# ShamG1/marl-traffic-intersection

Hardware: AMD Instinct MI355X
Metric: agent-steps/sec (whole node) at 4096 envs × 8 agents × 64-beam lidar; 1/2/4/8 GPU (higher is better)
Workload: dtype f32

## Files before the change

marl-traffic-intersection_amd/csrc/mev_kernels.hip:

```cpp
#include <type_traits>

#include <cstdlib>

#include "mev_kernels.h"
#include "mev_world.h"
#include "mev_nsort.h"

namespace mev {

#ifdef MEV_STAMPS
#define STAMP_RAW(k)                                                     \
    do {                                                                 \
        __builtin_amdgcn_wave_barrier();                                 \
        if (threadIdx.x == 0) p.debug[e * 8 + (k)] = __builtin_amdgcn_s_memtime(); \
    } while (0)
#if defined(MEV_STAMPS_R)
#undef STAMP_RAW
#define STAMP_RAW(k)                                                     \
    do {                                                                 \
        __builtin_amdgcn_wave_barrier();                                 \
        if (threadIdx.x == 0) p.debug[e * 8 + (k)] = __builtin_amdgcn_s_memrealtime(); \
    } while (0)
#ifndef MEV_STAMPS_POSTEND
#define MEV_STAMPS_POSTEND 0
// ... 2041 lines not shown
                                  float iady, float rwm, float ccen, float crf) {
    const float big = 1.0e6f;
    const float rx = fx - 375.0f, ry = fy - 375.0f;
    const float ax = fabs_f(rx), ay = fabs_f(ry);
    const float sx = ax < rwm ? rwm * iadx - rx * idx : 0.0f;
    const float sy = ay < rwm ? rwm * iady - ry * idy : 0.0f;
    const float sqm = ccen - 1.55f, rg = crf + 2.0f;
    const float qx = rx != 0.0f ? rx : dx, qy = ry != 0.0f ? ry : dy;
    const float ocx = rx - (qx >= 0.0f ? ccen : -ccen), ocy = ry - (qy >= 0.0f ? ccen : -ccen);
    const float bq = ocx * dx + ocy * dy;
    const float cq = ocx * ocx + ocy * ocy - rg * rg;
    const float disc = bq * bq - cq;
    const float troot = lidar_keep(-bq - __builtin_amdgcn_sqrtf(disc));
    const float tdisc = cq <= 0.0f ? 0.0f : ((disc < 0.0f || bq >= 0.0f) ? big : troot);
    const float tsq = fminf(sqm * iadx - rx * idx, sqm * iady - ry * idy);
    const float tq = fminf(rx * dx < 0.0f ? -rx * idx : big, ry * dy < 0.0f ? -ry * idy : big);
    const float sc = fmaxf(ax, ay) < sqm ? fminf(tdisc, fminf(tsq, tq)) : 0.0f;
    const float road = fmaxf(fmaxf(sx, sy), sc);
    const float tx = (dx > 0.0f ? 748.5f - fx : fx - 0.5f) * iadx;
    const float ty = (dy > 0.0f ? 748.5f - fy : fy - 0.5f) * iady;
    return fminf(road, fminf(tx, ty));
}

__device__ inline float road_safe_uniform(float fx, float fy, float dx, float dy, float idx, float idy, float iadx,
                                          float iady, float rwm, float ccen, float crf) {
    const float big = 1.0e6f;
    const float rx = fx - 375.0f, ry = fy - 375.0f;
    const float ax = fabs_f(rx), ay = fabs_f(ry);
    const float sqm = ccen - 1.55f, rg = crf + 2.0f;
    float road = 0.0f;
    if (__builtin_amdgcn_readfirstlane((int)(ax < rwm))) road = fmaxf(road, rwm * iadx - rx * idx);
    if (__builtin_amdgcn_readfirstlane((int)(ay < rwm))) road = fmaxf(road, rwm * iady - ry * idy);
    if (__builtin_amdgcn_readfirstlane((int)(fmaxf(ax, ay) < sqm))) {
        const float qx = rx != 0.0f ? rx : dx, qy = ry != 0.0f ? ry : dy;
        const float ocx = rx - (qx >= 0.0f ? ccen : -ccen), ocy = ry - (qy >= 0.0f ? ccen : -ccen);
        const float bq = ocx * dx + ocy * dy;
        const float cq = ocx * ocx + ocy * ocy - rg * rg;
        const float disc = bq * bq - cq;
        const float troot = lidar_keep(-bq - __builtin_amdgcn_sqrtf(disc));
        const float tdisc = cq <= 0.0f ? 0.0f : ((disc < 0.0f || bq >= 0.0f) ? big : troot);
        const float tsq = fminf(sqm * iadx - rx * idx, sqm * iady - ry * idy);
        const float tq = fminf(rx * dx < 0.0f ? -rx * idx : big, ry * dy < 0.0f ? -ry * idy : big);
        road = fmaxf(road, fminf(tdisc, fminf(tsq, tq)));
    }
    const float tx = (dx > 0.0f ? 748.5f - fx : fx - 0.5f) * iadx;
    const float ty = (dy > 0.0f ? 748.5f - fy : fy - 0.5f) * iady;
    return fminf(road, fminf(tx, ty));
}

__device__ inline float atan2_fast(float y, float x) {
    const float ax = fabs_f(x), ay = fabs_f(y);
    const float mx = fmaxf(ax, ay), mn = fminf(ax, ay);
    const float t = mn * __builtin_amdgcn_rcpf(fmaxf(mx, 1e-30f));
    const float s2 = t * t;
    float r = ((-0.0464964749f * s2 + 0.15931422f) * s2 - 0.327622764f) * s2 * t + t;
    r = ay > ax ? 1.57079637f - r : r;
    r = x < 0.0f ? 3.14159274f - r : r;
    return y < 0.0f ? -r : r;
}

__device__ inline float wrap_pi_fast(float a) { return a - 6.28318531f * rintf(a * 0.159154943f); }

__device__ inline float box_lo(int lo) { return (float)(lo > 0 ? lo : lo - 1) - 0.01f; }
__device__ inline float box_hi(int hi) { return (float)hi + 1.01f; }

__device__ inline void slab_clip(float c0, float dc, float idc, float a, float b, float& lo, float& hi) {
    if (fabs_f(dc) < 1e-6f) {
        if (c0 < a || c0 > b) { lo = 1.0f; hi = 0.0f; }
        return;
    }
    const float t1 = (a - c0) * idc, t2 = (b - c0) * idc;
    lo = fmaxf(lo, fminf(t1, t2));
    hi = fminf(hi, fmaxf(t1, t2));
}




#ifndef MEV_LIDAR_NPR
#define MEV_LIDAR_NPR 2
#endif
constexpr int LIDAR_NPR = MEV_LIDAR_NPR;
constexpr int kMarchHelp = 16;
constexpr int kNptHelp = 3;
static_assert(kMarchHelp <= 32, "helper groups have at least 2 lanes");

int lidar_group(int R) {
    int g = 256 / (R > 0 ? R : 1);
    return g < 1 ? 1 : (g > 64 ? 64 : g);
}

struct LidarSrcHbm {
    static constexpr bool kBoxLds = false;
    const SimParams& p;
    __device__ float rel(int b) const { return gmem(p.rel_angles)[b]; }
    __device__ bool alive(int g) const { return gmem(p.ego.alive)[g] != 0; }
    __device__ float4 pose(int g) const { return make_float4(egof(p, EF_X)[g], egof(p, EF_Y)[g], egof(p, EF_H)[g], __int_as_float(g)); }
    __device__ void cand(int g, unsigned long long& c0, unsigned long long& c1) const {
        c0 = gmem(p.ob_cand)[2 * g];
        c1 = gmem(p.ob_cand)[2 * g + 1];
    }
    __device__ int4 box(int g, int o) const { return p.ob_box[(size_t)(g / p.N) * p.ob_stride + o]; }
};
struct LidarSrcLds {
    static constexpr bool kBoxLds = true;
    const CarsLDS& el;
    int g0;
    __device__ float rel(int b) const { return el.rel[b]; }
    __device__ bool alive(int g) const { return el.alive[g - g0] != 0; }
    __device__ float4 pose(int g) const {
        const int i = g - g0;
        return make_float4(el.x[i], el.y[i], el.h[i], __int_as_float(g));
    }
    __device__ void cand(int g, unsigned long long& c0, unsigned long long& c1) const {
        c0 = el.cand[2 * (g - g0)];
        c1 = el.cand[2 * (g - g0) + 1];
    }
    __device__ int4 box(int, int o) const { return el.box[o]; }
};
template <int ENVS>
struct LidarSrcLdsEnvs {
    static constexpr bool kBoxLds = true;
    const CarsLDS& el0;
    int reg;
    const float* relp;
    int env[ENVS];
    __device__ int off(int g) const {
        int j = 0;
#pragma unroll
        for (int u = 1; u < ENVS; ++u) j = g == env[u] ? u : j;
        return j * reg;
    }
    template <class T>
    __device__ const T* at(const T* p0, int g) const {
        return reinterpret_cast<const T*>(reinterpret_cast<const unsigned char*>(p0) + off(g));
    }
    __device__ float rel(int b) const { return relp[b]; }
    __device__ bool alive(int g) const { return at(el0.alive, g)[0] != 0; }
    __device__ float4 pose(int g) const {
        return make_float4(at(el0.x, g)[0], at(el0.y, g)[0], at(el0.h, g)[0], __int_as_float(g));
    }
    __device__ void cand(int g, unsigned long long& c0, unsigned long long& c1) const {
        const unsigned long long* c = at(el0.cand, g);
        c0 = c[0];
        c1 = c[1];
    }
    __device__ int4 box(int g, int o) const { return at(el0.box, g)[o]; }
};

#ifndef MEV_DENSE_ILP
#define MEV_DENSE_ILP 2
#endif
template <bool TAB, int ILP, class Src, int NPT = LIDAR_NPR, bool HELP = false, int PART = 0, int P1 = 0,
          bool WC = false>
__device__ __forceinline__ void lidar_body(const SimParams& p, const Outputs& out, const Src& src, const int G,
                                           const int a0, const int na, const int lane, unsigned char* base,
                                           const LidarLayout& lay, const unsigned long long redo = 0ull,
                                           const unsigned long long alive_in = 0ull) {
    static_assert(!WC || (!TAB && P1 >= WAVE), "the reference's world: no distance table, the beams at compile time");
    using W = StepWorld<WC>;
    using RW = StepRows<WC, P1>;
    const int R = P1 >= WAVE ? P1 : p.R;
    const int LS = P1 >= WAVE ? P1 : p.lidar_slots;
    float4* ag = reinterpret_cast<float4*>(base + lay.ag);
    float2* dir = reinterpret_cast<float2*>(base + lay.dir);
    int* res = reinterpret_cast<int*>(base + lay.res);
#if defined(MEV_STAMPS_R)
    const int se_ = a0 / p.N, sp_ = ((a0 % p.N) / G) & 1;
    if (lane == 0) p.debug[se_ * 8 + 3 + sp_] = __builtin_amdgcn_s_memrealtime();
#endif

    bool alv = false;
    if (PART != 0) alv = (alive_in >> lane) & 1ull;
    else if (lane < na) alv = src.alive(a0 + lane);
    const unsigned long long am = PART != 0 ? alive_in : ballot(alv);
    const int nal = __popcll(am);
    if (PART == 0 && alv) {
        const int g = a0 + lane;
        ag[lane_rank(am)] = src.pose(g);
    }
    if (PART != 2 && __popcll(am) != na) {
        for (int j = 0; j < na; ++j) {
            if ((am >> j) & 1ull) continue;
            if (RW::lidar_u8(out)) {
                uint8_t* crow = RW::lidar_u8(out) + (size_t)(a0 + j) * LS;
                for (int b = lane; b < LS; b += WAVE) crow[b] = (uint8_t)kLidarCodeDead;
                continue;
            }
            float* row = out.obs + (size_t)(a0 + j) * RW::obs_ld(out) + OBS_HEAD;
            for (int b = lane; b < LS; b += WAVE) row[b] = 0.0f;
        }
    }
    wave_lds_sync();
    const float stp = W::lidar_step(p);
    const int S = W::lidar_steps(p);
    const float rwf = (float)W::irw(p);
    const float inv_stp = __builtin_amdgcn_rcpf(stp);
    const float crf = CORNER_RADIUS, ccen = rwf + crf;
    const float cr2p1 = crf * crf + 1.0f;
    const float rwm = rwf - 1.5f;
    auto probe = [&](float cx_, float cy_, float dx_, float dy_, int k_, float& fx, float& fy) -> int {
        const bool past = k_ >= S;
        const int kc = past ? S - 1 : k_;
        const float d = TAB ? gmem(p.dist_tab)[kc] : (float)kc * stp;
        fx = cx_ + dx_ * d;
        fy = cy_ + dy_ * d;
        const int px = (int)fx, py = (int)fy;
        const unsigned pmax = (unsigned)px > (unsigned)py ? (unsigned)px : (unsigned)py;
        const bool off_screen = pmax >= (unsigned)WIDTH;
        const float iax = fabs_f((float)(px - 375)), iay = fabs_f((float)(py - 375));
        const float qdx = iax - ccen, qdy = iay - ccen;
        const float onv = fmaxf(fminf(fminf(iax, iay) - rwf, fmaxf(iax, iay) - ccen), cr2p1 - (qdx * qdx + qdy * qdy));
        const bool stop = off_screen | ((k_ > 0) & (onv > 0.0f));
        const int code = lidar_keep(stop ? ((k_ << 1) | (off_screen ? 0 : 1)) : -1);
        return past ? (S << 1) : code;
    };
    auto probes_n = [&](auto np, float cx_, float cy_, float dx_, float dy_, int k_, float& fx, float& fy) -> int {
        int r = -1;
#pragma unroll
        for (int t = 0; t < decltype(np)::value; ++t) {
            const int c = probe(cx_, cy_, dx_, dy_, k_ + t, fx, fy);
            r = r >= 0 ? r : c;
        }
        return r;
    };
    auto probes = [&](float cx_, float cy_, float dx_, float dy_, int k_, float& fx, float& fy) -> int {
        return probes_n(std::integral_constant<int, LIDAR_NPR>{}, cx_, cy_, dx_, dy_, k_, fx, fy);
    };

    unsigned short* queue = reinterpret_cast<unsigned short*>(base + lay.queue);
    int qn = 0;
    const float rel_c0 = lane < R ? src.rel(lane) : 0.0f;
    const float rel_c1 = lane + WAVE < R ? src.rel(lane + WAVE) : 0.0f;
    auto setup = [&](const float4& a, float rel_b, auto small, float2& d, bool uni) -> int {
        float sn, cs;
#if defined(MEV_EXP_FASTSIN)
        sn = __sinf(a.z + rel_b);
        cs = __cosf(a.z + rel_b);
        (void)small;
#else
        if constexpr (decltype(small)::value) sincosf_below120(a.z + rel_b, &sn, &cs);
        else sincosf(a.z + rel_b, &sn, &cs);
#endif
        const float dx = cs, dy = -sn;
        d = make_float2(dx, dy);
        const int px = (int)a.x, py = (int)a.y;
        const unsigned pmax = (unsigned)px > (unsigned)py ? (unsigned)px : (unsigned)py;
        const float idx = __builtin_amdgcn_rcpf(dx), idy = __builtin_amdgcn_rcpf(dy);
        float safe;
        if (uni)
            safe = road_safe_uniform(a.x, a.y, dx, dy, idx, idy, fabs_f(idx), fabs_f(idy), rwm, ccen, crf);
        else
            safe = road_safe(a.x, a.y, dx, dy, idx, idy, fabs_f(idx), fabs_f(idy), rwm, ccen, crf);
        const int k1 = pmax < (unsigned)WIDTH ? 1 + safe_steps(safe, stp, inv_stp) : 0;
        float fx, fy;
        const int r = probes_n(std::integral_constant<int, LIDAR_NPR>{}, a.x, a.y, dx, dy, k1, fx, fy);
        return r >= 0 ? r : -(k1 + LIDAR_NPR) - 1;
    };
    auto pass1_one = [&](auto small, const int j) {
        const float4 a = ag[j];
        for (int b0 = 0; b0 < R; b0 += WAVE) {
            const int b = b0 + lane;
            const bool vb = b < R;
            const float rel_b = b0 == 0 ? rel_c0 : (b0 == WAVE ? rel_c1 : (vb ? src.rel(b) : 0.0f));
            float2 d;
            const int r = setup(a, rel_b, small, d, true);
            if (vb) {
                dir[j * R + b] = d;
                res[j * R + b] = r >= 0 ? r : -r - 1;
            }
            const bool pend = vb && r < 0;
            const unsigned long long m = ballot(pend);
            if (pend) queue[qn + lane_rank(m)] = (unsigned short)(j * R + b);
            qn += __popcll(m);
        }
    };
    const bool dense = P1 >= WAVE ? (P1 & (WAVE - 1)) != 0 : (P1 == 2 || (P1 == 0 && (R & (WAVE - 1)) != 0 && nal > 1));
    auto phase1 = [&](auto small) {
        if constexpr (PART == 2) {
            for (unsigned long long tm = redo; tm; tm &= tm - 1ull) pass1_one(small, __builtin_ctzll(tm));
        } else if (dense) {
            const float invRp = 1.0f / (float)R;
            const int nq = nal * R;
            constexpr int DI = ILP > 1 ? MEV_DENSE_ILP : 1;
            for (int c0 = 0; c0 < nq; c0 += DI * WAVE) {
                if (PART == 0 && 4 * c0 >= nq) __builtin_amdgcn_s_setprio(kPrioP1B);
                int q[DI];
                float4 a[DI];
                float rb[DI];
#pragma unroll
                for (int u = 0; u < DI; ++u) {
                    q[u] = c0 + u * WAVE + lane;
                    const int qc = q[u] < nq ? q[u] : nq - 1;
                    const int j = (int)(((float)qc + 0.5f) * invRp);
                    a[u] = ag[j];
                    rb[u] = src.rel(qc - j * R);
                }
                float2 d[DI];
                int r[DI];
#pragma unroll
                for (int u = 0; u < DI; ++u) r[u] = setup(a[u], rb[u], small, d[u], false);
#pragma unroll
                for (int u = 0; u < DI; ++u) {
                    const bool vq = q[u] < nq;
                    if (vq) {
                        dir[q[u]] = d[u];
                        res[q[u]] = r[u] >= 0 ? r[u] : -r[u] - 1;
// ... 8 lines not shown
        for (int j = 0; j < nal; j += ILP) {
            if (PART == 0 && 4 * j >= nal) __builtin_amdgcn_s_setprio(kPrioP1B);
            float4 a[ILP];
#pragma unroll
            for (int u = 0; u < ILP; ++u) a[u] = ag[j + u < nal ? j + u : j];
            for (int b0 = 0; b0 < R; b0 += WAVE) {
                const int b = b0 + lane;
                const bool vb = b < R;
                const float rel_b = b0 == 0 ? rel_c0 : (b0 == WAVE ? rel_c1 : (vb ? src.rel(b) : 0.0f));
                float2 d[ILP];
                int r[ILP];
#pragma unroll
                for (int u = 0; u < ILP; ++u) r[u] = setup(a[u], rel_b, small, d[u], true);
#pragma unroll
                for (int u = 0; u < ILP; ++u) {
                    const bool in = j + u < nal;
                    if (vb && in) {
                        dir[(j + u) * R + b] = d[u];
                        res[(j + u) * R + b] = r[u] >= 0 ? r[u] : -r[u] - 1;
                    }
                    const bool pend = vb && in && r[u] < 0;
                    const unsigned long long m = ballot(pend);
                    if (pend) queue[qn + lane_rank(m)] = (unsigned short)((j + u) * R + b);
                    qn += __popcll(m);
                }
            }
        }
        }
    };
    const bool hsmall = ballot(lane < nal && !(fabs_f(ag[lane < nal ? lane : 0].z) < 100.0f)) == 0ull;
    if (ILP > 1 && hsmall) phase1(std::true_type{});
    else phase1(std::false_type{});
    wave_lds_sync();
#if defined(MEV_EXP_STOP) && MEV_EXP_STOP == 2
    if (Src::kBoxLds) return;
#endif
#if defined(MEV_STAMPS_R)
    if (lane == 0 && na == p.N) p.debug[se_ * 8 + 4] = __builtin_amdgcn_s_memrealtime();
#endif

    if (PART == 0) __builtin_amdgcn_s_setprio(kPrioP2);
#if defined(MEV_EXP_TSNOMARCH)
    if constexpr (PART == 1) return;
#endif
    const float invR = 1.0f / (float)R;
    int next = qn < WAVE ? qn : WAVE;
    int slot = lane < qn ? (int)queue[lane] : -1;
    float cx = 0.0f, cy = 0.0f, dx = 0.0f, dy = 0.0f, idx = 0.0f, idy = 0.0f, iadx = 0.0f, iady = 0.0f;
    int k = 0;
    auto load_beam = [&](int qq) {
        const int j = (int)(((float)qq + 0.5f) * invR);
        const float4 a = ag[j];
        const float2 d = dir[qq];
        cx = a.x; cy = a.y; dx = d.x; dy = d.y;
        idx = __builtin_amdgcn_rcpf(dx);
        idy = __builtin_amdgcn_rcpf(dy);
        iadx = fabs_f(idx);
        iady = fabs_f(idy);
        k = res[qq];
    };
    if (slot >= 0) load_beam(slot);
    int* hscr = reinterpret_cast<int*>(base + lay.scr);
    bool help = false;
    while (ballot(slot >= 0) != 0ull) {
        if (HELP && next >= qn && __popcll(ballot(slot >= 0)) <= kMarchHelp) {
            help = true;
            break;
        }
        const bool act = slot >= 0;
        float fx, fy;
        int r, npr = LIDAR_NPR;
        if (NPT != LIDAR_NPR && next >= qn) {
            r = probes_n(std::integral_constant<int, NPT>{}, cx, cy, dx, dy, k, fx, fy);
            npr = NPT;
        } else {
            r = probes(cx, cy, dx, dy, k, fx, fy);
        }
        const float safe = road_safe(fx, fy, dx, dy, idx, idy, iadx, iady, rwm, ccen, crf);
        const int kn = k + npr + safe_steps(safe, stp, inv_stp);
        const bool fin = act & ((r >= 0) | (kn >= S));
        if (fin) res[slot] = r >= 0 ? r : (S << 1);
        k = kn;
        const unsigned long long fm = ballot(fin);
        if (fm != 0ull) {
            if (fin) {
                const int nq = next + lane_rank(fm);
                slot = nq < qn ? (int)queue[nq] : -1;
                if (slot >= 0) load_beam(slot);
            }
            next += __popcll(fm);
        }
    }
    if (HELP && help) {
        constexpr int NPH = kNptHelp;
        const unsigned long long am = ballot(slot >= 0);
        const int nb = __popcll(am);
        if (slot >= 0) {
            const int rk = lane_rank(am);
            hscr[2 * rk] = slot;
            hscr[2 * rk + 1] = k;
        }
        wave_lds_sync();
        auto group_march = [&](auto gs_c) {
            constexpr int GS = decltype(gs_c)::value;
            const int gi = lane / GS, j = lane & (GS - 1);
            slot = gi < nb ? hscr[2 * gi] : -1;
            const int k_h = gi < nb ? hscr[2 * gi + 1] : 0;
            if (slot >= 0) load_beam(slot);
            k = k_h;
            while (ballot(slot >= 0) != 0ull) {
                float fx, fy;
                const int k0 = k + j * NPH;
                int r = probes_n(std::integral_constant<int, NPH>{}, cx, cy, dx, dy, k0, fx, fy);
                r = r >= 0 ? r : 0x7fffffff;
                const float safe = road_safe(fx, fy, dx, dy, idx, idy, iadx, iady, rwm, ccen, crf);
                int kn = k0 + NPH + safe_steps(safe, stp, inv_stp);
                r = min(r, __builtin_amdgcn_mov_dpp(r, 0xB1, 0xf, 0xf, false));
                if constexpr (GS == 2) {
                    kn = __builtin_amdgcn_mov_dpp(kn, 0xF5, 0xf, 0xf, false);
                } else {
                    r = min(r, __builtin_amdgcn_mov_dpp(r, 0x4E, 0xf, 0xf, false));
                    kn = __builtin_amdgcn_mov_dpp(kn, 0xFF, 0xf, 0xf, false);
                    if constexpr (GS == 8) {
                        r = min(r, __builtin_amdgcn_mov_dpp(r, 0x141, 0xf, 0xf, false));
                        const int km = __builtin_amdgcn_mov_dpp(kn, 0x141, 0xf, 0xf, false);
                        kn = j < 4 ? km : kn;
                    }
                }
                const bool fin = slot >= 0 && (r != 0x7fffffff || kn >= S);
                if (fin && j == 0) res[slot] = r != 0x7fffffff ? r : (S << 1);
                slot = fin ? -1 : slot;
                k = kn;
            }
        };
        if (nb <= 8) group_march(std::integral_constant<int, 8>{});
        else if (nb <= 16) group_march(std::integral_constant<int, 4>{});
        else group_march(std::integral_constant<int, 2>{});
    }
    wave_lds_sync();
    if constexpr (PART == 1) return;
#if defined(MEV_EXP_STOP) && MEV_EXP_STOP == 3
    if (Src::kBoxLds) return;
#endif
#if defined(MEV_STAMPS_R)
    if (lane == 0 && na == p.N) p.debug[se_ * 8 + 6] = __builtin_amdgcn_s_memrealtime();
#endif

    __builtin_amdgcn_s_setprio(kPrioP3);
    int* seg_jo = reinterpret_cast<int*>(base + lay.seg_jo);
    int4* seg_rg = reinterpret_cast<int4*>(base + lay.seg_rg);
    int4* seg_bx = reinterpret_cast<int4*>(base + lay.seg_bx);
    int* scr = reinterpret_cast<int*>(base + lay.scr);
    int M = 0;
    unsigned long long cl0 = 0ull, cl1 = 0ull;
    if (lane < nal) src.cand(__float_as_int(ag[lane].w), cl0, cl1);
    for (int j = 0; j < nal; ++j) {
        const unsigned long long c0 = readlane64(cl0, j), c1 = readlane64(cl1, j);
        const int n0 = __popcll(c0);
        if ((c0 >> lane) & 1ull) seg_jo[M + lane_rank(c0)] = (j << 8) | lane;
        if ((c1 >> lane) & 1ull) seg_jo[M + n0 + lane_rank(c1)] = (j << 8) | (lane + WAVE);
        M += n0 + __popcll(c1);
    }
    wave_lds_sync();
    const float rel0 = src.rel(0);
    const bool all_beams = R == 1 || !W::beam_cull(p);
    const float dphi = R > 1 ? (src.rel(R - 1) - rel0) / (float)(R - 1) : 1.0f;
    const float idphi = 1.0f / dphi;
    const float period = 6.28318531f * idphi;
    for (int m = lane; m < M; m += WAVE) {
        const int jo = seg_jo[m];
        const float4 a = ag[jo >> 8];
        const int4 bx = src.box(__float_as_int(a.w), jo & 255);
        if (!Src::kBoxLds) seg_bx[m] = bx;
        const float ex0 = box_lo(bx.x), ex1 = box_hi(bx.y);
        const float ey0 = box_lo(bx.z), ey1 = box_hi(bx.w);
        int4 rg;
        if (all_beams || (a.x >= ex0 && a.x <= ex1 && a.y >= ey0 && a.y <= ey1)) {
            rg = make_int4(0 | (R << 16), 0, 0, R);
        } else {
            const bool lx = a.x < ex0, hx = a.x > ex1, ly = a.y < ey0, hy = a.y > ey1;
            const bool mx = !lx && !hx, my = !ly && !hy;
            const float Xa = my ? (lx ? ex0 : ex1) : (mx ? ex0 : ((lx == ly) ? ex1 : ex0));
            const float Ya = my ? ey0 : (mx ? (ly ? ey0 : ey1) : ey0);
            const float Xb = my ? Xa : (mx ? ex1 : ((lx == ly) ? ex0 : ex1));
            const float Yb = my ? ey1 : (mx ? Ya : ey1);
            const float phc = atan2_fast(-(0.5f * (ey0 + ey1) - a.y), 0.5f * (ex0 + ex1) - a.x);
            const float da = wrap_pi_fast(atan2_fast(-(Ya - a.y), Xa - a.x) - phc);
            const float db = wrap_pi_fast(atan2_fast(-(Yb - a.y), Xb - a.x) - phc);
            const float dmin = fminf(0.0f, fminf(da, db)), dmax = fmaxf(0.0f, fmaxf(da, db));
            float w = phc + dmin - a.z - rel0;
            w -= 6.28318531f * floorf(w * 0.159154943f);
            const float marg = 2.0e-4f;
            const float ulo = (w - marg) * idphi, uhi = (w + (dmax - dmin) + marg) * idphi;
            int lo[3], cn[3];
#pragma unroll
            for (int sft = 0; sft < 3; ++sft) {
                const float sh = (float)(sft - 1) * period;
                int l0 = (int)ceilf(ulo + sh), l1 = (int)floorf(uhi + sh);
                l0 = l0 < 0 ? 0 : l0;
                l1 = l1 > R - 1 ? R - 1 : l1;
                lo[sft] = l0;
                cn[sft] = l1 >= l0 ? l1 - l0 + 1 : 0;
            }
            rg = make_int4(lo[0] | (cn[0] << 16), lo[1] | (cn[1] << 16), lo[2] | (cn[2] << 16), cn[0] + cn[1] + cn[2]);
        }
        seg_rg[m] = rg;
    }
    wave_lds_sync();
    for (int cb = 0; cb < M; cb += WAVE) {
        const int nseg = M - cb < WAVE ? M - cb : WAVE;
        const int cnt = lane < nseg ? seg_rg[cb + lane].w : 0;
        const int incl = wave_scan_add(cnt);
        const int excl = incl - cnt;
        const int T = __builtin_amdgcn_readlane(incl, WAVE - 1);
        int carry = 0;
        for (int q0 = 0; q0 < T; q0 += WAVE) {
            const int q = q0 + lane;
            const bool starts = cnt > 0 && excl >= q0 && excl < q0 + WAVE;
            scr[lane] = 0;
            wave_lds_sync();
            if (starts) scr[excl - q0] = ((excl << 8) | lane) + 1;
            wave_lds_sync();
            const int got = wave_scan_max(scr[lane]);
            wave_lds_sync();
            const int cur = got > 0 ? got - 1 : carry;
            carry = __builtin_amdgcn_readlane(cur, WAVE - 1);
            const int sm = cur & 255;
            const int r = q - (cur >> 8);
            if (q < T) {
                const int m = cb + sm;
                const int j = seg_jo[m] >> 8;
                const float4 a = ag[j];
                const int4 rg = seg_rg[m];
                const int4 bx = Src::kBoxLds ? src.box(__float_as_int(a.w), seg_jo[m] & 255) : seg_bx[m];
                const int cA = rg.x >> 16, cB = rg.y >> 16;
                const int b = r < cA ? (rg.x & 0xffff) + r
                                     : (r < cA + cB ? (rg.y & 0xffff) + r - cA : (rg.z & 0xffff) + r - cA - cB);
                const int slot = j * R + b;
                const int kr = res[slot] >> 1;
                const float2 dd = dir[slot];
                float lo = 0.0f, hi = 1.0e6f;
                slab_clip(a.x, dd.x, __builtin_amdgcn_rcpf(dd.x), box_lo(bx.x), box_hi(bx.y), lo, hi);
                slab_clip(a.y, dd.y, __builtin_amdgcn_rcpf(dd.y), box_lo(bx.z), box_hi(bx.w), lo, hi);
                int ka, kb;
                if (TAB) {
                    ka = (int)(fmaxf(lo, 0.0f) * inv_stp) - 1;
                    kb = (int)(fminf(hi, 1.0e6f) * inv_stp) + 1;
                } else {
                    ka = (int)ceilf(fmaxf(lo, 0.0f) * inv_stp);
                    kb = (int)(fminf(hi, 1.0e6f) * inv_stp);
                }
                ka = ka < 1 ? 1 : ka;
                kb = kb < kr - 1 ? kb : kr - 1;
                if (lo > hi) kb = 0;
                for (int kk = ka; kk <= kb; ++kk) {
                    const float d = p.dist_tab ? gmem(p.dist_tab)[kk] : (float)kk * W::lidar_step(p);
                    const int px = (int)(a.x + dd.x * d), py = (int)(a.y + dd.y * d);
                    if (px >= bx.x && px <= bx.y && py >= bx.z && py <= bx.w) {
                        atomicMin(&res[slot], (kk << 1) | 1);
                        break;
                    }
                }
            }
        }
    }
    wave_lds_sync();
#if defined(MEV_STAMPS_R)
    if (lane == 0) p.debug[se_ * 8 + 5 + sp_] = __builtin_amdgcn_s_memrealtime();
#endif
#if defined(MEV_EXP_STOP) && MEV_EXP_STOP == 4
    if (Src::kBoxLds) return;
#endif
    if (RW::lidar_u8(out)) {
        for (int j = 0; j < nal; ++j) {
            const int g = __float_as_int(ag[j].w);
            uint8_t* crow = RW::lidar_u8(out) + (size_t)g * LS;
            for (int b = lane; b < LS; b += WAVE) {
                const int r = res[j * R + b];
                crow[b] = (uint8_t)((r & 1) ? (r >> 1) + 1 : 0);
            }
        }
        return;
    }
    if (LS <= WAVE) {
        const int gl = lane < nal ? __float_as_int(ag[lane].w) : 0;
        const bool beam = lane < LS;
        float l_max = W::lidar_max(p), l_step = W::lidar_step(p), l_inv = W::lidar_inv(p);
        if constexpr (!WC) asm volatile("" : "+v"(l_max), "+v"(l_step), "+v"(l_inv));
        auto row_value = [&](int r) {
            const float dk = TAB ? gmem(p.dist_tab)[r >> 1] : (float)(r >> 1) * l_step;
            return ((r & 1) ? dk : l_max) * l_inv;
        };
        for (int j0 = 0; j0 < nal; j0 += 8) {
            int rr[8];
#pragma unroll
            for (int u = 0; u < 8; ++u) rr[u] = (j0 + u < nal && beam) ? res[(j0 + u) * R + lane] : 0;
#pragma unroll
            for (int u = 0; u < 8; ++u) {
                if (j0 + u < nal && beam) {
                    const int g = __builtin_amdgcn_readlane(gl, j0 + u);
                    obs_store<true>(&out.obs[(size_t)g * RW::obs_ld(out) + OBS_HEAD + lane], row_value(rr[u]));
                }
            }
        }
    } else {
        for (int j = 0; j < nal; ++j) {
            const int g = __float_as_int(ag[j].w);
            float* row = out.obs + (size_t)g * RW::obs_ld(out) + OBS_HEAD;
            for (int b = lane; b < LS; b += WAVE)
                obs_store<true>(row + b, ((res[j * R + b] & 1) ? march_dist<TAB, WC>(p, res[j * R + b] >> 1) : W::lidar_max(p)) *
                                             W::lidar_inv(p));
        }
    }
}

template <bool TAB>
__global__ __launch_bounds__(256, 8) void k_lidar(SimParams p, Outputs out, int G, int a_begin, int a_end) {
    extern __shared__ __align__(16) unsigned char lds_raw[];
    const int lane = threadIdx.x & (WAVE - 1);
    const int wv = threadIdx.x / WAVE;
    const int blk = xcd_env((int)blockIdx.x, (int)gridDim.x);
    const int a0 = __builtin_amdgcn_readfirstlane(a_begin + (blk * (int)(blockDim.x / WAVE) + wv) * G);
    if (a0 >= a_end) return;
    const int na = a_end - a0 < G ? a_end - a0 : G;
    __builtin_amdgcn_s_setprio(kPrioLidar);
    const LidarLayout lay = lidar_layout(G, p.R, lidar_cand_max(p));
    lidar_body<TAB, 1>(p, out, LidarSrcHbm{p}, G, a0, na, lane, lds_raw + (size_t)wv * (size_t)lay.bytes, lay);
}


template <int NM, int KM>
__host__ __device__ inline StepLayout step_layout_t(const SimParams& p) {
    if constexpr (NM == 0) return step_layout(p);
    else return StepLayout{FixedLayout<NM, KM>::rel, FixedLayout<NM, KM>::rel, FixedLayout<NM, KM>::envw,
                           FixedLayout<NM, KM>::lidar, FixedLayout<NM, KM>::bytes};
}
#ifndef MEV_PHASE1_ILP
#define MEV_PHASE1_ILP 2
#endif
#ifndef MEV_ESPLIT_ILP
#define MEV_ESPLIT_ILP 1
#endif
constexpr int kPhase1Ilp = MEV_PHASE1_ILP;
constexpr int kEsplitIlp = MEV_ESPLIT_ILP;

template <bool TRAFFIC>
__device__ __forceinline__ void deal_append(const SimParams& p, const StepInputs& in, const CarsCtx& cx, const int e) {
    if constexpr (TRAFFIC) {
        if (!(in.deal & 2)) return;
        const int lane0 = threadIdx.x & (WAVE - 1);
        const int x = (int)blockIdx.x & (kDealLists - 1);
        const int nxt = in.deal_ring == 2 ? 0 : in.deal_ring + 1;
        if (lane0 == 0) {
            const int c = (in.auto_reset && cx.ended) ? 0 : (cx.ncnt < kDealClasses - 1 ? cx.ncnt : kDealClasses - 1);
            const int slot = atomicAdd(p.deal_cnt + (size_t)nxt * kDealRingInts + (x * kDealClasses + c) * kDealPad, 1);
            const size_t ring_off = (size_t)nxt * kDealLists * kDealClasses * (size_t)p.E;
            gmem(p.deal_order)[ring_off + ((size_t)x * kDealClasses + c) * p.E + slot] = e;
        }
        if (blockIdx.x == 0 && lane0 < kDealLists * kDealClasses) {
            const int clr = nxt == 2 ? 0 : nxt + 1;
            gmem(p.deal_cnt)[(size_t)clr * kDealRingInts + lane0 * kDealPad] = 0;
        }
    }
}

constexpr int kSplitWpe = 4;
constexpr int kEsplitWpe = 8;
#ifndef MEV_TSPLIT_LPRIO
#define MEV_TSPLIT_LPRIO 1
#endif
constexpr int kPrioTsplitLidar = MEV_TSPLIT_LPRIO;
constexpr int kTsplitWpe = 6;
constexpr int kPrioEsplitRoad = 3;
constexpr int kPrioEsplitCars = 2;
#ifndef MEV_TSPLIT_CPRIO
#define MEV_TSPLIT_CPRIO kPrioEsplitCars
#endif
constexpr int kPrioTsplitCars = MEV_TSPLIT_CPRIO;
constexpr int kPrioEsplitCarPhase = 1;
template <bool TRAFFIC, bool TAB, int NM, int KM = MAXK, int PK = 1, bool SPLIT = false, bool ESPLIT = false, int P1 = 0,
          int NC = 0, bool WC = false>
__global__ __launch_bounds__((TRAFFIC && ESPLIT) ? (PK + 1) * WAVE : (SPLIT ? 2 * WAVE : WAVE),
                             (TRAFFIC && ESPLIT) ? kTsplitWpe
                                                 : ((ESPLIT && PK == 1) ? kEsplitWpe : (SPLIT ? kSplitWpe : 4))) void k_step(
    const SimParams* __restrict__ pp, StepInputs in, Outputs out) {
#include "mev_step_body.inc"
}

template <bool TRAFFIC, bool TAB, int NM, int KM, bool SPLIT, int SP1 = 0, int SNC = 0>
__global__ __launch_bounds__(SPLIT ? 2 * WAVE : WAVE, SPLIT ? kSplitWpe : 4) void k_serve(
    const SimParams* __restrict__ pp, ServeArgs sa, Outputs out) {
    __shared__ uint32_t cmdw[kServeLine];
    constexpr int PK = 1;
    constexpr bool ESPLIT = false;
    constexpr int P1 = SP1, NC = SNC;
    constexpr bool WC = false;
    const int lane = threadIdx.x & (WAVE - 1);
    const bool w0 = threadIdx.x < WAVE;
    ServeBox* box = sa.box;
    uint32_t last_seq = 0xffffffffu;
    uint32_t served = __builtin_amdgcn_readfirstlane(
        __hip_atomic_load(&box->done[blockIdx.x], __ATOMIC_ACQUIRE, __HIP_MEMORY_SCOPE_SYSTEM));
    for (;;) {
        if (w0) {
            const uint64_t t0 = __builtin_amdgcn_s_memrealtime();
            uint32_t seq = last_seq, quit = 0u;
            for (;;) {
                seq = __builtin_amdgcn_readfirstlane(
                    __hip_atomic_load(&box->seq, __ATOMIC_ACQUIRE, __HIP_MEMORY_SCOPE_SYSTEM));
                if (seq != last_seq) break;
                if (__builtin_amdgcn_s_memrealtime() - t0 > sa.idle_ticks) {
                    quit = 1u;
                    break;
                }
                __builtin_amdgcn_s_sleep(4);
            }
            uint32_t word = 0u;
            if (lane < kServeLine) word = __hip_atomic_load(&box->seq + lane, __ATOMIC_RELAXED, __HIP_MEMORY_SCOPE_SYSTEM);
// ... 294 lines not shown
```

marl-traffic-intersection_amd/csrc/mev_layout.h:

```cpp
#pragma once

#include <stddef.h>
#include <stdint.h>

#if !defined(__HIPCC__) && !defined(__host__)
#define __host__
#define __device__
#endif

namespace mev {

constexpr int WAVE = 64;
constexpr int MAXN = 64;
constexpr int MAXK = 64;

template <int KM, bool DIMS = false>
struct NpcLDST {
    static constexpr bool kDims = DIMS;
    static constexpr int kCap = KM;
    float x[KM], y[KM], v[KM], h[KM], c[KM], s[KM], acc[KM], steer[KM];
    int32_t pidx[KM], route[KM], intent[KM];
    uint8_t alive[KM];
    union {
        struct {
            float cx[KM][4], cy[KM][4];
        };
        struct {
            float xn[KM], yn[KM], vn[KM], hn[KM], accn[KM], steern[KM], cn[KM], sn[KM];
            float mdcn[KM];
        };
    };
    unsigned long long col[KM];
    float thr_a[KM], thr_b[KM];
    unsigned long long em[KM], ym[KM];
    unsigned long long em_a[KM], ym_a[KM];
    float mc_a[KM];
    int32_t pidxn[KM];
    int32_t pidx0[KM];
    float nsteer[KM], ntan[KM];
    float accb[KM], mdc[KM];
    float endx[KM], endy[KM];
    float len[DIMS ? KM : 0], wid[DIMS ? KM : 0];
};

constexpr int kWinBytes = 5 * 1024;

__host__ __device__ constexpr size_t lds_al(size_t b) { return (b + 15) & ~size_t(15); }

template <class P>
__host__ __device__ inline int cars_k(const P& p) { return p.traffic ? p.K : 0; }

__host__ __device__ constexpr size_t cars_lds_bytes(int N, int K, bool dims = false) {
    const size_t n = (size_t)N, ob = (size_t)(N + K);
    return 22 * lds_al(n * 4) + 2 * lds_al(n * 16) + 3 * lds_al(n * 4) + 4 * lds_al(n) + lds_al(n * 8) +
           lds_al(ob * 16) + 3 * lds_al(ob * 4) + lds_al(n * 16) + (dims ? 2 * lds_al(n * 4) : 0);
}

struct LidarLayout {
    int ag, dir, res, seg_jo, seg_rg, seg_bx, queue, scr, bytes;
};

template <class P>
__host__ __device__ inline int lidar_cand_max(const P& p) { return p.N - 1 + (p.traffic ? p.K : 0); }

__host__ __device__ constexpr LidarLayout lidar_layout_beams(int G, int beams, int cmax, bool with_bx) {
    LidarLayout L{};
    const int C = G * cmax;
    int off = 0;
    L.ag = off; off += G * 16;
    L.dir = off; off += beams * 8;
    L.res = off; off += beams * 4;
    off = (off + 15) & ~15;
    L.seg_rg = off; off += C * 16;
    L.seg_bx = off; off += with_bx ? C * 16 : 0;
    L.seg_jo = off; off += C * 4;
    L.queue = L.seg_rg;
    if (off < L.queue + beams * 2) off = L.queue + beams * 2;
    off = (off + 15) & ~15;
    L.scr = off; off += WAVE * 4;
    L.bytes = (off + 15) & ~15;
    return L;
}
__host__ __device__ inline LidarLayout lidar_layout(int G, int R, int cmax, bool with_bx = true) {
    return lidar_layout_beams(G, G * R, cmax, with_bx);
}

__host__ __device__ constexpr int step_pool_n(int N, int R) {
    int g = 512 / (R > 0 ? R : 1);
    g = g < 1 ? 1 : g;
    if (g >= N) return N;
    const int pools = (N + g - 1) / g;
    return (N + pools - 1) / pools;
}
template <class P>
__host__ __device__ inline int step_pool(const P& p) { return step_pool_n(p.N, p.R); }

struct StepLayout {
    int head, rel, envw, lidar, bytes;
};
template <class P>
__host__ __device__ inline StepLayout step_layout(const P& p) {
    StepLayout L;
    int off = (int)lds_al(cars_lds_bytes(p.N, cars_k(p), true));
    L.head = off;
    L.rel = off; off += (int)lds_al((size_t)p.R * 4);
    L.envw = off; off += 32;
    L.lidar = off; off += lidar_layout(step_pool(p), p.R, lidar_cand_max(p), false).bytes;
    L.bytes = off;
    return L;
}

constexpr int kFixedRays = 128;
constexpr int kPoolBeams = 512;
template <int NM, int KM = 0>
struct FixedLayout {
    static_assert(NM >= 1 && NM <= 64, "agents per env");
    static constexpr int beams = NM * kFixedRays < kPoolBeams ? NM * kFixedRays : kPoolBeams;
    static constexpr int cars = (int)lds_al(cars_lds_bytes(NM, KM));
    static constexpr int rel = cars;
    static constexpr int envw = rel + kFixedRays * 4;
    static constexpr int lidar = envw + 32;
    static constexpr LidarLayout lay = lidar_layout_beams(NM, beams, NM - 1 + KM, false);
    static constexpr int bytes = lidar + lay.bytes;
};

#ifndef MEV_TSPLIT_ENVS
#define MEV_TSPLIT_ENVS 2
#endif
constexpr int kTsplitEnvs = MEV_TSPLIT_ENVS;
constexpr int kTsplitRays = kFixedRays;

}
```

marl-traffic-intersection_amd/csrc/mev_step_body.inc:

```
    static_assert(!SPLIT || !TRAFFIC || ESPLIT, "split waves with traffic: the early split");
    static_assert(!WC || (!TRAFFIC && !TAB && NM > 0 && PK == 1 && !SPLIT && P1 >= WAVE && NC > 0),
                  "the world at compile time: one wave per env, the counts at compile time, no table");
    const SimParams& p = *pp;
    extern __shared__ __align__(16) unsigned char step_lds[];
    const int wv = SPLIT ? __builtin_amdgcn_readfirstlane((int)(threadIdx.x >> 6)) : 0;
    int npc_cls = kDealClasses - 1;
    const int e = (TRAFFIC && (in.deal & 1)) ? deal_env(p, in.deal_ring, (int)blockIdx.x, 1, 0, &npc_cls)
                                             : xcd_env((int)blockIdx.x, (int)gridDim.x) * PK;
#if defined(MEV_STAMPS_R)
    STAMP_RAW(0);
#endif
    QSTAMP(0);
    constexpr int KF = TRAFFIC ? KM : 0;
    constexpr int NCE = NM == 1 ? 1 : NC;
    const StepLayout sl = step_layout_t<NM, KF>(p);
    constexpr bool DIMS = NM == 0;
    using NLT = NpcLDST<KM, DIMS>;
    CarsLDS el = NM ? carve_cars_lds(step_lds, NM, KF) : carve_cars_lds(step_lds, p.N, cars_k(p), DIMS);
    el.head = reinterpret_cast<float*>(step_lds + sl.head);
    el.rel = reinterpret_cast<float*>(step_lds + sl.rel);
    el.envw = reinterpret_cast<int32_t*>(step_lds + sl.envw);
    if constexpr (!TRAFFIC && NM > 0) {
        static_assert(NM == 0 || FixedLayout<(NM ? NM : 1), 0>::lay.bytes >= kWinBytes, "LDS path windows");
        el.win = reinterpret_cast<float4*>(step_lds + sl.lidar);
    }
    __shared__ typename std::conditional<TRAFFIC, NLT, char>::type nl_storage[(TRAFFIC && ESPLIT) ? PK : 1];
    NLT* nl = nullptr;
    if constexpr (TRAFFIC) nl = &nl_storage[0];
    __builtin_amdgcn_s_setprio(kPrioCars);
    if constexpr (TRAFFIC && ESPLIT) {
        static_assert(SPLIT && NM == 1 && KF > 0, "traffic early split: one ego per env, compile-time layout");
        constexpr int REG = FixedLayout<1, KF>::lidar;
        const int lane = threadIdx.x & (WAVE - 1);
        const int b = (int)blockIdx.x;
        if (wv < PK) {
            int cls = kDealClasses - 1;
            const int ej = (in.deal & 1) ? deal_env(p, in.deal_ring, b, PK, wv, &cls) : xcd_env(b, (int)gridDim.x) * PK + wv;
            unsigned char* rb = step_lds + wv * REG;
            CarsLDS elj = carve_cars_lds(rb, 1, KF);
            elj.head = reinterpret_cast<float*>(rb + sl.head);
            elj.rel = reinterpret_cast<float*>(rb + sl.rel);
            elj.envw = reinterpret_cast<int32_t*>(rb + sl.envw);
            NLT* nlj = &nl_storage[wv];
            __builtin_amdgcn_s_setprio(kPrioTsplitCars);
            CarsCtx cx = cars_pre<true, true, NLT, 1, false, true, false, true, NCE>(p, in, out, ej, elj, nlj, cls);
            cars_post<true, true, NLT, 1, false, NCE>(p, out, ej, elj, nlj, cx);
            deal_append<true>(p, in, cx, ej);
#if defined(MEV_STAMPS_Q)
            QSTAMP(7);
            if (lane == 0)
                for (int q = 0; q < 8; ++q) p.debug[ej * 8 + q] = mev_qst[wv * 8 + q];
#endif
            return;
        }
        __builtin_amdgcn_s_setprio(kPrioTsplitLidar);
        int es[PK];
#pragma unroll
        for (int j = 0; j < PK; ++j)
            es[j] = (in.deal & 1) ? deal_env(p, in.deal_ring, b, PK, j) : xcd_env(b, (int)gridDim.x) * PK + j;
        unsigned char* lbase = step_lds + PK * REG;
        constexpr LidarLayout lay = lidar_layout_beams(PK, PK * kTsplitRays, KF, false);
        float* rel0 = reinterpret_cast<float*>(step_lds + sl.rel);
        for (int bb = lane; bb < p.R; bb += WAVE) rel0[bb] = gmem(p.rel_angles)[bb];
        const unsigned long long am = ts_ego_phase<PK, KF>(p, in, step_lds, REG, es, lane);
        const bool on = lane < PK;
        const bool alive = ((am >> lane) & 1ull) != 0;
        int ee = es[0];
#pragma unroll
        for (int j = 1; j < PK; ++j) ee = lane == j ? es[j] : ee;
        for (unsigned long long dm = ballot(on && !alive); dm; dm &= dm - 1ull) {
            const int g = __builtin_amdgcn_readlane(ee, __builtin_ctzll(dm));
            if (out.lidar_u8) {
                for (int bb = lane; bb < p.lidar_slots; bb += WAVE)
                    out.lidar_u8[(size_t)g * p.lidar_slots + bb] = (uint8_t)kLidarCodeDead;
            } else {
                for (int bb = lane; bb < p.lidar_slots; bb += WAVE) out.obs[(size_t)g * out.obs_ld + OBS_HEAD + bb] = 0.0f;
            }
        }
        float4* ag = reinterpret_cast<float4*>(lbase + lay.ag);
        if (alive) {
            const CarsLDS elp = carve_cars_lds(step_lds + lane * REG, 1, KF);
            ag[lane_rank(am)] = make_float4(elp.x[0], elp.y[0], elp.h[0], __int_as_float(ee));
        }
        wave_lds_sync();
        const CarsLDS el0 = carve_cars_lds(step_lds, 1, KF);
        LidarSrcLdsEnvs<PK> src{el0, REG, rel0, {}};
#pragma unroll
        for (int j = 0; j < PK; ++j) src.env[j] = es[j];
        const int nal = __popcll(am);
        lidar_body<TAB, kEsplitIlp, LidarSrcLdsEnvs<PK>, LIDAR_NPR, true, 1, P1>(p, out, src, PK, 0, nal, lane, lbase,
                                                                             lay, 0ull, am);
        __syncthreads();
        __syncthreads();
        const int li = on ? lane : 0;
        const bool rs = alive && (reinterpret_cast<const int32_t*>(step_lds + li * REG + sl.envw)[6] & 1) != 0;
        const unsigned long long rl = ballot(rs);
        unsigned long long redo = 0ull;
        if (rl != 0ull) {
            if (rs) {
                const CarsLDS elr = carve_cars_lds(step_lds + li * REG, 1, KF);
                ag[lane_rank(am)] = make_float4(elr.x[0], elr.y[0], elr.h[0], __int_as_float(ee));
            }
            for (unsigned long long m = rl; m; m &= m - 1ull) {
                const int i = __builtin_ctzll(m);
                redo |= 1ull << __popcll(am & ((1ull << i) - 1ull));
            }
            wave_lds_sync();
        }
        __builtin_amdgcn_s_setprio(kPrioEsplitCarPhase);
        lidar_body<TAB, kEsplitIlp, LidarSrcLdsEnvs<PK>, LIDAR_NPR, true, 2, P1>(p, out, src, PK, 0, nal, lane, lbase,
                                                                             lay, redo, am);
        return;
    } else if constexpr (ESPLIT) {
        static_assert(SPLIT && !TRAFFIC && NM > 0, "early split without traffic: two waves");
        const int lane = threadIdx.x & (WAVE - 1);
        const int NE = NCE ? NCE : p.N;
        const int g0 = e * NE;
        const int NS = PK == 1 ? NE : (p.E - e < PK ? p.E - e : PK) * NE;
        unsigned char* lbase = step_lds + sl.lidar;
        const LidarLayout lay = FixedLayout<(NM ? NM : 1), 0>::lay;
        if (wv == 0) {
            __builtin_amdgcn_s_setprio(kPrioEsplitCars);
            CarsCtx cx = cars_pre<false, true, NLT, PK, false, true, false, false, NCE>(p, in, out, e, el, nl);
            cars_post<false, true, NLT, PK, false, NCE>(p, out, e, el, nl, cx);
        } else {
            __builtin_amdgcn_s_setprio(kPrioEsplitRoad);
            for (int b = lane; b < p.R; b += WAVE) el.rel[b] = gmem(p.rel_angles)[b];
            const bool on = lane < NS;
            const int il = on ? lane : 0;
            const int ee = PK == 1 ? e : e + il / NE;
            const uint32_t ug = (uint32_t)(g0 + il);
            const bool pend = ldu(gmem(p.pending_reset), (uint32_t)ee) != 0;
            const int route_l = ldu(egoi(p, EF_ROUTE), ug);
            Kin k{ldu(egof(p, EF_X), ug), ldu(egof(p, EF_Y), ug), ldu(egof(p, EF_V), ug), ldu(egof(p, EF_H), ug),
                  ldu(egof(p, EF_ACC), ug), ldu(egof(p, EF_STEER), ug)};
            bool alive = ldu(gmem(p.ego.alive), ug) != 0;
            const float a0 = ldu(gmem(in.actions), 2 * ug), a1 = ldu(gmem(in.actions), 2 * ug + 1);
            if (in.auto_reset && pend) {
                const int rid = reset_route(p, in.rng_counter, ee, PK == 1 ? il : il - (ee - e) * NE, route_l);
                k = Kin{gmem(p.rt.spawn)[3 * rid], gmem(p.rt.spawn)[3 * rid + 1], 0.0f, gmem(p.rt.spawn)[3 * rid + 2],
                        0.0f, 0.0f};
                alive = true;
            }
            {
                Kin ku = k;
                float sH, cH;
                car_update_heading(ku, a0, a1, in.dt);
                sincosf(alive ? ku.h : k.h, &sH, &cH);
                car_update_move(ku, cH, sH);
                if (alive) k = ku;
            }
            alive = on && alive;
            const unsigned long long am = ballot(alive);
            float4* ag = reinterpret_cast<float4*>(lbase + lay.ag);
            if (alive) ag[lane_rank(am)] = make_float4(k.x, k.y, k.h, __int_as_float(g0 + il));
            wave_lds_sync();
            lidar_body<TAB, kEsplitIlp, LidarSrcLds, LIDAR_NPR, true, 1, P1>(
                p, out, LidarSrcLds{el, g0}, NS, g0, NS, lane, lbase, lay, 0ull, am);
            __syncthreads();
            const unsigned rmask = (unsigned)el.envw[6];
            const bool rs = alive && lane < 32 && ((rmask >> (lane & 31)) & 1u);
            const unsigned long long rl = ballot(rs);
            unsigned long long redo = 0ull;
            if (rl != 0ull) {
                if (rs) ag[lane_rank(am)] = make_float4(el.x[lane], el.y[lane], el.h[lane], __int_as_float(g0 + lane));
                for (unsigned long long m = rl; m; m &= m - 1ull) {
                    const int i = __builtin_ctzll(m);
                    redo |= 1ull << __popcll(am & ((1ull << i) - 1ull));
                }
                wave_lds_sync();
            }
            __builtin_amdgcn_s_setprio(kPrioEsplitCarPhase);
            lidar_body<TAB, kEsplitIlp, LidarSrcLds, LIDAR_NPR, true, 2, P1>(
                p, out, LidarSrcLds{el, g0}, NS, g0, NS, lane, lbase, lay, redo, am);
        }
        return;
    }
    if constexpr (!(TRAFFIC && ESPLIT)) {
    CarsCtx cx{};
    if (wv == 0) cx = cars_pre<TRAFFIC, true, NLT, PK, (!TRAFFIC && NM > 0), false, DIMS, false, NCE, false, WC>(p, in, out, e, el, nl, npc_cls);
    if (SPLIT) __syncthreads();
    else wave_lds_sync();
#if !defined(MEV_EXP_STOP) || MEV_EXP_STOP != 0
    if (wv == 0) {
        cars_post<TRAFFIC, true, NLT, PK, DIMS, NCE, false, (WC ? P1 : 0)>(p, out, e, el, nl, cx);
        wave_lds_sync();
    }
#endif
    deal_append<TRAFFIC>(p, in, cx, e);
#if defined(MEV_EXP_STOP) && MEV_EXP_STOP == 0
    return;
#endif
    if (SPLIT && wv == 0) return;
#if defined(MEV_EXP_STOP) && MEV_EXP_STOP == 1
    return;
#endif
    const int NEC = NCE ? NCE : p.N;
    const int NS = PK == 1 ? NEC : (p.E - e < PK ? p.E - e : PK) * NEC;
    int G = 512 / (p.R > 0 ? p.R : 1);
    G = G < 1 ? 1 : (G < NS ? G : NS);
    if (PK == 1) G = (NCE > 0 && P1 >= WAVE) ? step_pool_n(NCE, P1) : step_pool(p);
    const LidarLayout lay = NM ? FixedLayout<(NM ? NM : 1), KF>::lay : lidar_layout(G, p.R, lidar_cand_max(p), false);
    unsigned char* lbase = step_lds + sl.lidar;
    const int lane = threadIdx.x & (WAVE - 1);
    const int g0 = e * NEC;
    for (int j0 = 0; j0 < NS; j0 += G) {
        if (j0 > 0) wave_lds_sync();
        if (j0 > 0) __builtin_amdgcn_s_setprio(kPrioLidar);
        const int na = NS - j0 < G ? NS - j0 : G;
        lidar_body<TAB, kPhase1Ilp, LidarSrcLds, LIDAR_NPR, true, 0, P1, WC>(
            p, out, LidarSrcLds{el, g0}, G, g0 + j0, na, lane, lbase, lay);
    }
#if defined(MEV_STAMPS_Q)
    QSTAMP(7);
    if ((threadIdx.x & 63) == 0)
        for (int q = 0; q < 8; ++q) p.debug[e * 8 + q] = mev_qst[wv * 8 + q];
#endif
#if defined(MEV_STAMPS_R)
    if (!SPLIT || wv == 1) {
        const unsigned long long t = __builtin_amdgcn_s_memrealtime() & ((1ull << 40) - 1);
        const unsigned hw = __builtin_amdgcn_s_getreg((15 << 11) | 4) & 0xffffu;
        const unsigned xcc = __builtin_amdgcn_s_getreg((3 << 11) | 20) & 7u;
        if (lane == 0) p.debug[e * 8 + 7] = t | ((unsigned long long)(hw | (xcc << 16)) << 40);
    }
#endif
    }
```

Baseline: 1.178 billion.

## Map agent-box segments directly to lanes for 8-agent no-traffic lidar

For the 8-agent, no-traffic configuration, the lidar box-probe phase gives each lane one (agent, box) pair (lane>>3 picks the agent, lane&7 the box) and marks it active from the candidate mask. This replaces the serial per-agent candidate compaction loop into seg_jo and the chunked segment loop, leaving a single ballot plus one scan over up to 64 segments. It removes LDS round-trips and per-agent readlane iterations. The cost is idle lanes for inactive pairs and reliance on exactly 8 boxes per environment. Optional debug counters for segment statistics are added as well.

```diff
diff --git a/marl-traffic-intersection_amd/csrc/mev_kernels.hip b/marl-traffic-intersection_amd/csrc/mev_kernels.hip
--- a/marl-traffic-intersection_amd/csrc/mev_kernels.hip
+++ b/marl-traffic-intersection_amd/csrc/mev_kernels.hip
@@ -2217,7 +2217,7 @@
 #define MEV_DENSE_ILP 2
 #endif
 template <bool TAB, int ILP, class Src, int NPT = LIDAR_NPR, bool HELP = false, int PART = 0, int P1 = 0,
-          bool WC = false>
+          bool WC = false, bool SEGL = false>
 __device__ __forceinline__ void lidar_body(const SimParams& p, const Outputs& out, const Src& src, const int G,
                                            const int a0, const int na, const int lane, unsigned char* base,
                                            const LidarLayout& lay, const unsigned long long redo = 0ull,
@@ -2532,6 +2532,10 @@
     int4* seg_bx = reinterpret_cast<int4*>(base + lay.seg_bx);
     int* scr = reinterpret_cast<int*>(base + lay.scr);
     int M = 0;
+#if defined(MEV_SEG_COUNTS)
+    int dbg_t = 0, dbg_pass = 0;
+#endif
+    if constexpr (!SEGL) {
     unsigned long long cl0 = 0ull, cl1 = 0ull;
     if (lane < nal) src.cand(__float_as_int(ag[lane].w), cl0, cl1);
     for (int j = 0; j < nal; ++j) {
@@ -2542,11 +2546,131 @@
         M += n0 + __popcll(c1);
     }
     wave_lds_sync();
+    }
     const float rel0 = src.rel(0);
     const bool all_beams = R == 1 || !W::beam_cull(p);
     const float dphi = R > 1 ? (src.rel(R - 1) - rel0) / (float)(R - 1) : 1.0f;
     const float idphi = 1.0f / dphi;
     const float period = 6.28318531f * idphi;
+    if constexpr (SEGL) {
+        static_assert(std::is_same<Src, LidarSrcLds>::value, "segments by lane: one box table in the wave's LDS");
+        auto seg_range = [&](const float4& a, const int4& bx) -> int4 {
+            const float ex0 = box_lo(bx.x), ex1 = box_hi(bx.y);
+            const float ey0 = box_lo(bx.z), ey1 = box_hi(bx.w);
+            int4 rg;
+            if (all_beams || (a.x >= ex0 && a.x <= ex1 && a.y >= ey0 && a.y <= ey1)) {
+                rg = make_int4(0 | (R << 16), 0, 0, R);
+            } else {
+                const bool lx = a.x < ex0, hx = a.x > ex1, ly = a.y < ey0, hy = a.y > ey1;
+                const bool mx = !lx && !hx, my = !ly && !hy;
+                const float Xa = my ? (lx ? ex0 : ex1) : (mx ? ex0 : ((lx == ly) ? ex1 : ex0));
+                const float Ya = my ? ey0 : (mx ? (ly ? ey0 : ey1) : ey0);
+                const float Xb = my ? Xa : (mx ? ex1 : ((lx == ly) ? ex0 : ex1));
+                const float Yb = my ? ey1 : (mx ? Ya : ey1);
+                const float phc = atan2_fast(-(0.5f * (ey0 + ey1) - a.y), 0.5f * (ex0 + ex1) - a.x);
+                const float da = wrap_pi_fast(atan2_fast(-(Ya - a.y), Xa - a.x) - phc);
+                const float db = wrap_pi_fast(atan2_fast(-(Yb - a.y), Xb - a.x) - phc);
+                const float dmin = fminf(0.0f, fminf(da, db)), dmax = fmaxf(0.0f, fmaxf(da, db));
+                float w = phc + dmin - a.z - rel0;
+                w -= 6.28318531f * floorf(w * 0.159154943f);
+                const float marg = 2.0e-4f;
+                const float ulo = (w - marg) * idphi, uhi = (w + (dmax - dmin) + marg) * idphi;
+                int lo[3], cn[3];
+#pragma unroll
+                for (int sft = 0; sft < 3; ++sft) {
+                    const float sh = (float)(sft - 1) * period;
+                    int l0 = (int)ceilf(ulo + sh), l1 = (int)floorf(uhi + sh);
+                    l0 = l0 < 0 ? 0 : l0;
+                    l1 = l1 > R - 1 ? R - 1 : l1;
+                    lo[sft] = l0;
+                    cn[sft] = l1 >= l0 ? l1 - l0 + 1 : 0;
+                }
+                rg = make_int4(lo[0] | (cn[0] << 16), lo[1] | (cn[1] << 16), lo[2] | (cn[2] << 16), cn[0] + cn[1] + cn[2]);
+            }
+            return rg;
+        };
+        auto pair_probe = [&](const float4& a, const int4& rg, const int4& bx, const int j, const int r) {
+            const int cA = rg.x >> 16, cB = rg.y >> 16;
+            const int b = r < cA ? (rg.x & 0xffff) + r
+                                 : (r < cA + cB ? (rg.y & 0xffff) + r - cA : (rg.z & 0xffff) + r - cA - cB);
+            const int slot = j * R + b;
+            const int kr = res[slot] >> 1;
+            const float2 dd = dir[slot];
+            float lo = 0.0f, hi = 1.0e6f;
+            slab_clip(a.x, dd.x, __builtin_amdgcn_rcpf(dd.x), box_lo(bx.x), box_hi(bx.y), lo, hi);
+            slab_clip(a.y, dd.y, __builtin_amdgcn_rcpf(dd.y), box_lo(bx.z), box_hi(bx.w), lo, hi);
+            int ka, kb;
+            if (TAB) {
+                ka = (int)(fmaxf(lo, 0.0f) * inv_stp) - 1;
+                kb = (int)(fminf(hi, 1.0e6f) * inv_stp) + 1;
+            } else {
+                ka = (int)ceilf(fmaxf(lo, 0.0f) * inv_stp);
+                kb = (int)(fminf(hi, 1.0e6f) * inv_stp);
+            }
+            ka = ka < 1 ? 1 : ka;
+            kb = kb < kr - 1 ? kb : kr - 1;
+            if (lo > hi) kb = 0;
+            for (int kk = ka; kk <= kb; ++kk) {
+                const float d = p.dist_tab ? gmem(p.dist_tab)[kk] : (float)kk * W::lidar_step(p);
+                const int px = (int)(a.x + dd.x * d), py = (int)(a.y + dd.y * d);
+                if (px >= bx.x && px <= bx.y && py >= bx.z && py <= bx.w) {
+                    atomicMin(&res[slot], (kk << 1) | 1);
+                    break;
+                }
+            }
+        };
+        const int sj = lane >> 3, so = lane & 7;
+        bool seg = false;
+        float4 sa = make_float4(0.0f, 0.0f, 0.0f, 0.0f);
+        int4 sbx = make_int4(0, 0, 0, 0);
+        if (sj < nal) {
+            sa = ag[sj];
+            sbx = src.box(0, so);
+            unsigned long long c0, c1;
+            src.cand(__float_as_int(sa.w), c0, c1);
+            seg = (((unsigned)c0 >> so) & 1u) != 0u;
+        }
+        const unsigned long long segs = ballot(seg);
+        M = __popcll(segs);
+        if (segs != 0ull) {
+            int cnt = 0;
+            if (seg) {
+                const int4 rg = seg_range(sa, sbx);
+                seg_rg[lane] = rg;
+                cnt = rg.w;
+            }
+            wave_lds_sync();
+            const int incl = wave_scan_add(cnt);
+            const int excl = incl - cnt;
+            const int T = __builtin_amdgcn_readlane(incl, WAVE - 1);
+#if defined(MEV_SEG_COUNTS)
+            dbg_t = T;
+#endif
+            int carry = 0;
+            for (int q0 = 0; q0 < T; q0 += WAVE) {
+                const int q = q0 + lane;
+                const bool starts = cnt > 0 && excl >= q0 && excl < q0 + WAVE;
+                scr[lane] = 0;
+                wave_lds_sync();
+                if (starts) scr[excl - q0] = ((excl << 8) | lane) + 1;
+                wave_lds_sync();
+                const int got = wave_scan_max(scr[lane]);
+                wave_lds_sync();
+                const int cur = got > 0 ? got - 1 : carry;
+                carry = __builtin_amdgcn_readlane(cur, WAVE - 1);
+                const int sm = cur & 255;
+#if defined(MEV_SEG_COUNTS)
+                ++dbg_pass;
+#endif
+                if (q < T) {
+                    const float4 a = ag[sm >> 3];
+                    const int4 rg = seg_rg[sm];
+                    const int4 bx = src.box(0, sm & 7);
+                    pair_probe(a, rg, bx, sm >> 3, q - (cur >> 8));
+                }
+            }
+        }
+    } else {
     for (int m = lane; m < M; m += WAVE) {
         const int jo = seg_jo[m];
         const float4 a = ag[jo >> 8];
@@ -2607,6 +2731,9 @@
             carry = __builtin_amdgcn_readlane(cur, WAVE - 1);
             const int sm = cur & 255;
             const int r = q - (cur >> 8);
+#if defined(MEV_SEG_COUNTS)
+            ++dbg_pass;
+#endif
             if (q < T) {
                 const int m = cb + sm;
                 const int j = seg_jo[m] >> 8;
@@ -2643,7 +2770,19 @@
                 }
             }
         }
-    }
+#if defined(MEV_SEG_COUNTS)
+        dbg_t += T;
+#endif
+    }
+    }
+#if defined(MEV_SEG_COUNTS)
+    if (lane == 0) {
+        unsigned long long* dbg = p.debug + (size_t)(a0 / p.N) * 8 + 3 * (((a0 % p.N) / G) & 1);
+        dbg[0] = (unsigned long long)M;
+        dbg[1] = (unsigned long long)dbg_t;
+        dbg[2] = (unsigned long long)dbg_pass;
+    }
+#endif
     wave_lds_sync();
 #if defined(MEV_STAMPS_R)
     if (lane == 0) p.debug[se_ * 8 + 5 + sp_] = __builtin_amdgcn_s_memrealtime();
diff --git a/marl-traffic-intersection_amd/csrc/mev_layout.h b/marl-traffic-intersection_amd/csrc/mev_layout.h
--- a/marl-traffic-intersection_amd/csrc/mev_layout.h
+++ b/marl-traffic-intersection_amd/csrc/mev_layout.h
@@ -123,6 +123,9 @@
     static constexpr LidarLayout lay = lidar_layout_beams(NM, beams, NM - 1 + KM, false);
     static constexpr int bytes = lidar + lay.bytes;
 };
+static_assert(FixedLayout<8>::lay.seg_bx == FixedLayout<8>::lay.seg_jo &&
+                  FixedLayout<8>::lay.seg_rg + WAVE * 16 <= FixedLayout<8>::lay.scr,
+              "segments by lane: 64 ranges between seg_rg and scr");
 
 #ifndef MEV_TSPLIT_ENVS
 #define MEV_TSPLIT_ENVS 2
diff --git a/marl-traffic-intersection_amd/csrc/mev_step_body.inc b/marl-traffic-intersection_amd/csrc/mev_step_body.inc
--- a/marl-traffic-intersection_amd/csrc/mev_step_body.inc
+++ b/marl-traffic-intersection_amd/csrc/mev_step_body.inc
@@ -12,6 +12,7 @@
 #endif
     QSTAMP(0);
     constexpr int KF = TRAFFIC ? KM : 0;
+    constexpr bool SEGL = NM == 8 && KF == 0;
     constexpr int NCE = NM == 1 ? 1 : NC;
     const StepLayout sl = step_layout_t<NM, KF>(p);
     constexpr bool DIMS = NM == 0;
@@ -155,7 +156,7 @@
             float4* ag = reinterpret_cast<float4*>(lbase + lay.ag);
             if (alive) ag[lane_rank(am)] = make_float4(k.x, k.y, k.h, __int_as_float(g0 + il));
             wave_lds_sync();
-            lidar_body<TAB, kEsplitIlp, LidarSrcLds, LIDAR_NPR, true, 1, P1>(
+            lidar_body<TAB, kEsplitIlp, LidarSrcLds, LIDAR_NPR, true, 1, P1, false, SEGL>(
                 p, out, LidarSrcLds{el, g0}, NS, g0, NS, lane, lbase, lay, 0ull, am);
             __syncthreads();
             const unsigned rmask = (unsigned)el.envw[6];
@@ -171,7 +172,7 @@
                 wave_lds_sync();
             }
             __builtin_amdgcn_s_setprio(kPrioEsplitCarPhase);
-            lidar_body<TAB, kEsplitIlp, LidarSrcLds, LIDAR_NPR, true, 2, P1>(
+            lidar_body<TAB, kEsplitIlp, LidarSrcLds, LIDAR_NPR, true, 2, P1, false, SEGL>(
                 p, out, LidarSrcLds{el, g0}, NS, g0, NS, lane, lbase, lay, redo, am);
         }
         return;
@@ -208,7 +209,7 @@
         if (j0 > 0) wave_lds_sync();
         if (j0 > 0) __builtin_amdgcn_s_setprio(kPrioLidar);
         const int na = NS - j0 < G ? NS - j0 : G;
-        lidar_body<TAB, kPhase1Ilp, LidarSrcLds, LIDAR_NPR, true, 0, P1, WC>(
+        lidar_body<TAB, kPhase1Ilp, LidarSrcLds, LIDAR_NPR, true, 0, P1, WC, SEGL>(
             p, out, LidarSrcLds{el, g0}, G, g0 + j0, na, lane, lbase, lay);
     }
 #if defined(MEV_STAMPS_Q)
```

Result: faster. 1.259 billion (median of 6 runs) (+6.9%).
